# felixyu7/perceiver-io-1

Measured on AMD Instinct MI355X. Metric: samples/sec (whole node) IMDB MLM seq_len=512 at 1/2/4/8 MI355X, higher is better.
Workload: dtype bf16; 1 GPU; mlm256; model=perceiver-io-mlm latents=256x64 layers=3x(1+6) vocab=10003, global_batch=64, seq_len=512, parallelism=dp1, backend=hip, graph=True, allreduce_in_graph=False, bucket_update=False

## Files before the change

perceiver_io_amd/csrc/binding.cpp:

```cpp
#include <torch/extension.h>
#include <ATen/hip/HIPContext.h>
#include <hip/hip_runtime.h>

#include "host_api.h"

#include <tuple>
#include <unordered_map>
#include <vector>

using torch::Tensor;
using OptT = c10::optional<Tensor>;

namespace {
hipStream_t stream() { return at::hip::getCurrentHIPStream(); }

#ifndef PIO_CHECKS
#define PIO_CHECKS 0
#endif
int64_t check_errors(bool reset) {
  return (int64_t)(pio::check_errors_elementwise(reset) | pio::check_errors_optim(reset) |
                   pio::check_errors_mlm_head(reset) | pio::check_errors_mlm_select(reset) |
                   pio::check_errors_ce_head(reset) | pio::check_errors_topk_head(reset) |
                   pio::check_errors_rowgemm(reset) | pio::check_errors_pixel_head(reset) |
                   pio::check_errors_soft_ce_head(reset) | pio::check_errors_augment(reset) |
// ... 1401 lines not shown
  TORCH_CHECK(R > 0 && R < (int64_t(1) << 31), "text_kv_fwd: bad row count");
  TORCH_CHECK(la.size() == 4 && lb.size() == 4, "text_kv_fwd: [lnw, lnb, w, bias] per layer");
  auto opts = E.options();
  Tensor x = torch::empty({B, L, 64}, opts);
  Tensor mean = torch::empty({R}, opts), rstd = torch::empty({R}, opts);
  Tensor kva = torch::empty({R, 128}, opts.dtype(torch::kBFloat16)), kvb = torch::empty({R, 128}, opts.dtype(torch::kBFloat16));
  auto proj = [](std::vector<Tensor>& l, Tensor& kv) {
    TORCH_CHECK(l[0].is_contiguous() && l[0].numel() == 64 && l[1].is_contiguous() && l[1].numel() == 64,
                "text_kv_fwd: LN affine of 64 channels");
    TORCH_CHECK(l[2].dim() == 2 && l[2].is_contiguous() && l[2].size(0) == 128 && l[2].size(1) == 64,
                "text_kv_fwd: w must be (128, 64) contiguous");
    TORCH_CHECK(l[3].is_contiguous() && l[3].numel() == 128, "text_kv_fwd: bias of 128 columns");
    return pio::TextKvProj{f32p(l[0]), f32p(l[1]), bfp(l[2]), f32p(l[3]), bfp_mut(kv)};
  };
  pio::TextKvFwdArgs a{};
  a.ids = ids.data_ptr<int64_t>();
  a.E = f32p(E);
  a.P = f32p(P);
  a.scale = (float)scale;
  a.V = E.size(0);
  a.L = (int)L;
  a.R = (int)R;
  a.eps = (float)eps;
  a.a = proj(la, kva);
  a.b = proj(lb, kvb);
  a.X = x.data_ptr<float>();
  a.mean = mean.data_ptr<float>();
  a.rstd = rstd.data_ptr<float>();
  TORCH_CHECK(pio::text_kv_fwd_launch(a, stream()), "text_kv_fwd: operands must be 16-byte aligned");
  checked_sync("text_kv_fwd");
  return {x, mean, rstd, kva, kvb};
}

Tensor text_kv_bwd(Tensor ga, Tensor gb, Tensor x, Tensor mean, Tensor rstd, std::vector<Tensor> la,
                   std::vector<Tensor> lb, std::vector<Tensor> grads, bool slab, OptT job_slab,
                   std::vector<Tensor> job_dsts, std::vector<int64_t> job_offs) {
  CHECK_CUDA(ga); CHECK_CUDA(x);
  const int64_t R = ga.size(0);
  TORCH_CHECK(ga.dim() == 2 && ga.is_contiguous() && ga.size(1) == 128 && gb.is_contiguous() && gb.dim() == 2 &&
                  gb.size(0) == R && gb.size(1) == 128,
              "text_kv_bwd: dK|dV must be (R, 128) contiguous");
  TORCH_CHECK(x.is_contiguous() && x.numel() == R * 64 && mean.is_contiguous() && mean.numel() == R &&
                  rstd.is_contiguous() && rstd.numel() == R,
              "text_kv_bwd: x (R, 64) and its row statistics");
  TORCH_CHECK(R > 0 && R < kTallRows, "text_kv_bwd: bad row count");
  TORCH_CHECK(!g_det || slab, "deterministic mode: text_kv_bwd parameter gradients need slab mode");
  TORCH_CHECK(la.size() == 3 && lb.size() == 3 && grads.size() == 8, "text_kv_bwd: [lnw, lnb, w] per layer, 8 targets");
  const int64_t sr = slab ? (R + 63) / 64 : 0;
  int vrs = -1;
  auto layer = [&](const Tensor& g, std::vector<Tensor>& l, int t0) {
    TORCH_CHECK(l[0].is_contiguous() && l[0].numel() == 64 && l[1].is_contiguous() && l[1].numel() == 64,
                "text_kv_bwd: LN affine of 64 channels");
    TORCH_CHECK(l[2].dim() == 2 && l[2].is_contiguous() && l[2].size(0) == 128 && l[2].size(1) == 64,
                "text_kv_bwd: w must be (128, 64) contiguous");
    pio::TextKvGrad o{};
    o.G = f32p(g);
    o.lnw = f32p(l[0]);
    o.lnb = f32p(l[1]);
    o.W = bfp(l[2]);
    o.dlnw = vec_target(grads[t0], 64, "dlnw", vrs, sr);
    o.dlnb = vec_target(grads[t0 + 1], 64, "dlnb", vrs, sr);
    o.dW = vec_target(grads[t0 + 2], 128 * 64, "dW", vrs, sr);
    o.db = vec_target(grads[t0 + 3], 128, "db", vrs, sr);
    return o;
  };
  Tensor dx = torch::empty({R, 64}, ga.options());
  pio::TextKvBwdArgs a{};
  a.a = layer(ga, la, 0);
  a.b = layer(gb, lb, 4);
  a.X = f32p(x);
  a.mean = f32p(mean);
  a.rstd = f32p(rstd);
  a.dX = dx.data_ptr<float>();
  a.vrs = vrs < 0 ? 0 : vrs;
  a.slab = slab ? 1 : 0;
  a.R = (int)R;
  a.job = make_job(job_slab, job_dsts, job_offs);
  TORCH_CHECK(pio::text_kv_bwd_launch(a, stream()), "text_kv_bwd: operands must be 16-byte aligned");
  return dx;
}

void embed_bwd(Tensor ids, Tensor g, OptT dE, OptT dP, double scale, OptT job_slab, std::vector<Tensor> job_dsts,
               std::vector<int64_t> job_offs) {
  TORCH_CHECK(g.is_contiguous() && ids.is_contiguous());
  const pio::SlabJob job = make_job(job_slab, job_dsts, job_offs);
  const int B = (int)ids.size(0), L = (int)ids.size(1), C = (int)g.size(2);
  if (dE.has_value()) TORCH_CHECK(dE->is_contiguous() && dE->size(1) == C, "dE must be (V, C) contiguous");
  if (dP.has_value()) TORCH_CHECK(dP->is_contiguous() && dP->size(1) == C && dP->size(0) >= L, "dP must be (>= L, C)");
  if ((!dE.has_value() || dE->size(0) < (1 << 24)) &&
      pio::embed_bwd_local_launch(ids.data_ptr<int64_t>(), f32p(g), dE.has_value() ? dE->data_ptr<float>() : nullptr,
                                  dP.has_value() ? dP->data_ptr<float>() : nullptr, B, L, C, (float)scale, job,
                                  stream()))
    return;
  if (job.slab) pio::slab_reduce_launch(job, stream());
  if (dE.has_value()) {
    TORCH_CHECK(dE->is_contiguous() && dE->size(1) == C, "dE must be (V, C) contiguous");
    const bool small = dE->size(0) <= 32767;
    Tensor keys = small ? ids.reshape({-1}).to(torch::kInt16) : ids.reshape({-1});
    auto sorted = keys.sort();
    Tensor sid = std::get<0>(sorted).to(torch::kInt64).contiguous(), perm = std::get<1>(sorted).contiguous();
    pio::embed_bwd_sorted_launch(sid.data_ptr<int64_t>(), perm.data_ptr<int64_t>(), f32p(g), dE->data_ptr<float>(),
                                 ids.numel(), C, (float)scale, stream());
  }
  if (dP.has_value())
    pio::embed_bwd_launch(ids.data_ptr<int64_t>(), f32p(g), nullptr, dP->data_ptr<float>(), B, L, C, (float)scale,
                          stream());
}

std::vector<Tensor> text_mask(Tensor x, OptT pad, Tensor state, int64_t unk, int64_t mask, double p, int64_t lo,
// ... 802 lines not shown
        py::arg("pre") = std::vector<Tensor>{}, py::arg("post") = std::vector<Tensor>{});
  m.def("sb_bwd", &sb_bwd, py::arg("dz"), py::arg("x0"), py::arg("saved"), py::arg("params"),
        py::arg("scale"), py::arg("eps"), py::arg("pre") = std::vector<Tensor>{},
        py::arg("pre_saved") = std::vector<Tensor>{}, py::arg("zero_out") = py::none(),
        py::arg("post") = std::vector<Tensor>{}, py::arg("post_io") = std::vector<Tensor>{});
  m.def("sb_wgrad", &sb_wgrad, py::arg("jobs"), py::arg("job_slab") = py::none(),
        py::arg("job_dsts") = std::vector<Tensor>(), py::arg("job_offs") = std::vector<int64_t>());
  m.def("post_attn_ln_linear_fwd", &post_attn_ln_linear_fwd, py::arg("o"), py::arg("x"), py::arg("wo"), py::arg("bo"),
        py::arg("g2"), py::arg("be2"), py::arg("eps"), py::arg("w1"), py::arg("b1"), py::arg("w2"), py::arg("b2"),
        py::arg("lnw"), py::arg("lnb"), py::arg("wq"), py::arg("bq"), py::arg("seed") = py::none(),
        py::arg("site") = 0, py::arg("p") = 0.0);
  m.def("ln_linear_post_attn_bwd", &ln_linear_post_attn_bwd, py::arg("g"), py::arg("wq"), py::arg("x"),
        py::arg("mean1"), py::arg("rstd1"), py::arg("lnw"), py::arg("lnb"), py::arg("dres"), py::arg("ll_grads"),
        py::arg("y"), py::arg("m2"), py::arg("r2"), py::arg("u"), py::arg("o"), py::arg("wo"), py::arg("w1"),
        py::arg("w2"), py::arg("g2"), py::arg("be2"), py::arg("H"), py::arg("pa_grads"),
        py::arg("job_slab") = py::none(), py::arg("job_dsts") = std::vector<Tensor>(),
        py::arg("job_offs") = std::vector<int64_t>(), py::arg("seed") = py::none(), py::arg("site") = 0,
        py::arg("p") = 0.0, py::arg("zero_out") = py::none(), py::arg("att_qkv") = py::none(),
        py::arg("att_lse") = py::none(), py::arg("att_out") = py::none(), py::arg("att_scale") = 0.0);
  m.def("post_attn_bwd", &post_attn_bwd, py::arg("dz"), py::arg("y"), py::arg("m2"), py::arg("r2"), py::arg("u"),
        py::arg("o"), py::arg("wo"), py::arg("w1"), py::arg("w2"), py::arg("g2"), py::arg("be2"), py::arg("H"),
        py::arg("grads"), py::arg("slab") = false, py::arg("job_slab") = py::none(),
        py::arg("job_dsts") = std::vector<Tensor>(), py::arg("job_offs") = std::vector<int64_t>(),
        py::arg("seed") = py::none(), py::arg("site") = 0, py::arg("p") = 0.0, py::arg("zero_out") = py::none());
  m.def("ln_linear_bwd", &ln_linear_bwd, py::arg("g"), py::arg("w"), py::arg("x"), py::arg("mean"), py::arg("rstd"),
        py::arg("lnw"), py::arg("lnb"), py::arg("dres"), py::arg("need_dx"), py::arg("dlnw"), py::arg("dlnb"),
        py::arg("dW"), py::arg("db"), py::arg("pe") = py::none(), py::arg("kin") = -1, py::arg("slab") = false,
        py::arg("job_slab") = py::none(), py::arg("job_dsts") = std::vector<Tensor>(),
        py::arg("job_offs") = std::vector<int64_t>(), py::arg("dx_out") = py::none(), py::arg("pe_index") = py::none());
  m.def("text_kv_fwd", &text_kv_fwd, py::arg("ids"), py::arg("E"), py::arg("P"), py::arg("scale"), py::arg("eps"),
        py::arg("la"), py::arg("lb"));
  m.def("text_kv_bwd", &text_kv_bwd, py::arg("ga"), py::arg("gb"), py::arg("x"), py::arg("mean"), py::arg("rstd"),
        py::arg("la"), py::arg("lb"), py::arg("grads"), py::arg("slab") = false, py::arg("job_slab") = py::none(),
        py::arg("job_dsts") = std::vector<Tensor>(), py::arg("job_offs") = std::vector<int64_t>());
  m.def("wgrad", &wgrad, py::arg("g"), py::arg("a"), py::arg("amode"), py::arg("mean"), py::arg("rstd"), py::arg("lnw"),
        py::arg("lnb"), py::arg("rows_per_wg"), py::arg("dW"), py::arg("db"), py::arg("pe") = py::none(),
        py::arg("kin") = -1, py::arg("pe_index") = py::none());
  m.def("mlm_select", &mlm_select, py::arg("labels"), py::arg("cap"), py::arg("gcap"), py::arg("sticky") = py::none(),
        py::arg("queries") = py::none());
  m.def("index_add_rows", &index_add_rows);
  m.def("gather_rows", &gather_rows, py::arg("src"), py::arg("idx"));
  m.def("batch_sum2", &batch_sum2, py::arg("a"), py::arg("b"), py::arg("ob_acc") = py::none());
  m.def("pixel_ce_fwd", &pixel_ce_fwd);
  m.def("pixel_ce_bwd", &pixel_ce_bwd);
  m.def("pixel_predict", &pixel_predict, py::arg("h"), py::arg("w"), py::arg("b"), py::arg("qidx"), py::arg("qvalid"),
        py::arg("Q"), py::arg("npix"), py::arg("labels") = py::none());
  m.def("nonzero_compact", &nonzero_compact, py::arg("img"), py::arg("cap"), py::arg("segs") = 0, py::arg("tile") = 0);
  m.def("event_compact", &event_compact, py::arg("img"), py::arg("lab"), py::arg("words"), py::arg("key_cap"),
        py::arg("query_cap"), py::arg("wmask"), py::arg("ncls"), py::arg("segs") = 0, py::arg("tile") = 0);
  m.def("stage_step", &stage_step, py::arg("dsts"), py::arg("srcs"), py::arg("hyper_dst") = py::none(),
        py::arg("hyper") = std::vector<double>{}, py::arg("seed_dst") = py::none(),
        py::arg("seeds") = std::vector<int64_t>{});
  m.def("ce_fwd", &ce_fwd, py::arg("h"), py::arg("idx"), py::arg("labels"), py::arg("w"), py::arg("bias"),
        py::arg("count"), py::arg("zero_out") = py::none(), py::arg("count_labels") = false);
  m.def("ce_bwd", &ce_bwd, py::arg("h"), py::arg("labels"), py::arg("w"), py::arg("bias"),
        py::arg("lse"), py::arg("gout"), py::arg("count"), py::arg("dH"), py::arg("dW"), py::arg("db"),
        py::arg("accumulate"), py::arg("rowmap") = py::none(), py::arg("slab") = false, py::arg("u") = py::none(),
        py::arg("u_ml") = py::none());
  m.def("vocab_topk", &vocab_topk, py::arg("h"), py::arg("idx"), py::arg("w"), py::arg("bias"), py::arg("k"));
  m.def("soft_ce_fwd", &soft_ce_fwd, py::arg("h"), py::arg("label_a"), py::arg("label_b"), py::arg("lam"), py::arg("w"),
        py::arg("bias"), py::arg("eps"));
  m.def("soft_ce_bwd", &soft_ce_bwd, py::arg("hs"), py::arg("label_a"), py::arg("label_b"), py::arg("lam"), py::arg("w"),
        py::arg("bias"), py::arg("eps"), py::arg("lse"), py::arg("gout"), py::arg("count"), py::arg("dH"), py::arg("dW"),
        py::arg("db"), py::arg("accumulate"));
  m.def("batch_mix", &batch_mix, py::arg("x"), py::arg("y"), py::arg("mix"));
  m.def("batch_augment", &batch_augment, py::arg("src"), py::arg("params"), py::arg("mean"), py::arg("std"),
        py::arg("out_h"), py::arg("out_w"));
// ... 58 lines not shown
```

perceiver_io_amd/csrc/host_api.h:

```cpp
#pragma once
#include <stdint.h>

#include <hip/hip_runtime_api.h>

namespace pio {


struct AttnArgs {
  const uint16_t* q; long long q_bs; int q_rs;
  const uint16_t* k; long long k_bs; int k_rs;
  const uint16_t* v; long long v_bs; int v_rs;
  const uint8_t* kmask;
  int B, H, Nq, Nk;
  float scale_log2;
  float scale;
  uint32_t drop_thresh;
  float drop_scale;
  const int64_t* seedp;
  uint32_t site;
};

struct DropCfg {
  const int64_t* seed;
  uint32_t site;
// ... 104 lines not shown
  float *dlnw, *dlnb, *dW, *db;
  int vrs, wrs, slab;
  int R;
  PeSplit ps;
  SlabJob job;
};
struct TextKvProj {
  const float *lnw, *lnb;
  const uint16_t* W;
  const float* bias;
  uint16_t* KV;
};
struct TextKvFwdArgs {
  const int64_t* ids;
  const float *E, *P;
  float scale;
  long long V;
  int L, R;
  float eps;
  TextKvProj a, b;
  float *X, *mean, *rstd;
};
struct TextKvGrad {
  const float* G;
  const float *lnw, *lnb;
  const uint16_t* W;
  float *dlnw, *dlnb, *dW, *db;
};
struct TextKvBwdArgs {
  TextKvGrad a, b;
  const float *X, *mean, *rstd;
  float* dX;
  int vrs, slab, R;
  SlabJob job;
};
struct WgradArgs {
  RowsIn G; int N;
  RowsIn A; int Kin, amode;
  const float *mean, *rstd, *lnw, *lnb;
  int R;
  int rows_per_wg;
  float *dW, *db;
  int vrs, wrs;
  PeSplit ps;
};
struct PostAttnFwdArgs {
  const uint16_t* O;
  const float* X;
  PostAttnParams p;
  float* Z;
  PostAttnSaved s;
  int R, Rx;
  NextProj next;
  DropCfg dr;
};
struct SaLayerFwdArgs {
  const uint16_t* QKV;
  int N;
  float scale_log2;
  uint16_t* O;
  float* LSE;
  const float* X;
  PostAttnParams p;
  float* Z;
  PostAttnSaved s;
  int R;
// ... 202 lines not shown
                        float eps, uint16_t* y, float* mean, float* rstd, hipStream_t st);
int pe_proj_bwd_blocks(int M);
void pe_proj_bwd_launch(const float* dy, const float* pix, int nc, const float* mean, const float* rstd, int B, int M,
                        int O, float* D, float* part, hipStream_t st);
void persist_set_spin_limit(unsigned n);
unsigned persist_errors(bool reset);
int persist_sync_words(int B);
bool sa_block_fwd_launch(const SABlockFwdArgs& a, hipStream_t st);
int pixel_ce_blocks(long long R);
void pixel_ce_fwd_launch(int C, int K, const float* H, const float* W, const float* bias, const int64_t* labels,
                         const float* wts, long long R, float* part, float* stats, float* loss, hipStream_t st);
void pixel_ce_bwd_launch(int C, int K, const float* H, const float* W, const float* bias, const int64_t* labels,
                         const float* wts, const float* gout, const float* stats, long long R, float* dH, float* part,
                         float* dW, float* db, hipStream_t st);
void pixel_predict_launch(int C, int K, const float* H, const float* W, const float* bias, const int64_t* qidx,
                          const bool* qvalid, const int64_t* labels, long long R, long long Q, long long npix,
                          uint8_t* classes, float* conf, uint8_t* cmap, int* cpart, hipStream_t st);
void nonzero_compact_launch(const float* img, int B, long long npix, long long cap, int S, int V, int* segcount,
                            float* values, int64_t* index, bool* kmask, int* count, hipStream_t st);
unsigned check_errors_pixel_head(bool reset);
void rand_augment_launch(const uint8_t* src, const float* words, uint8_t* out, uint8_t* tmp, int* hist, int B, int H,
                         int W, int C, int N, int fill, hipStream_t st);
unsigned check_errors_randaugment(bool reset);
void ln_linear_fwd_launch(const LnLinearFwdArgs& a, hipStream_t st);
void post_attn_fwd_launch(const PostAttnFwdArgs& a, int C, hipStream_t st);
void post_attn_ln_linear_fwd_launch(const PostAttnFwdArgs& a, int C, hipStream_t st);
bool sa_layer_fwd_launch(const SaLayerFwdArgs& a, hipStream_t st);
void post_attn_bwd_launch(const PostAttnBwdArgs& a, int C, hipStream_t st);
bool ln_linear_post_attn_bwd_launch(const LnLinearPostAttnBwdArgs& a, int C, hipStream_t st);
void ln_linear_bwd_launch(const LnLinearBwdArgs& a, hipStream_t st);
void wgrad_launch(const WgradArgs& a, hipStream_t st);
bool text_kv_fwd_launch(const TextKvFwdArgs& a, hipStream_t st);
bool text_kv_bwd_launch(const TextKvBwdArgs& a, hipStream_t st);
unsigned check_errors_rowgemm(bool reset);
bool sb_fwd_launch(const SBFwdArgs& a, int C, hipStream_t st);
bool sb_bwd_launch(const SBBwdArgs& a, int C, hipStream_t st);
bool sb_wgrad_launch(SBWgradArgs a, int C, const SlabJob& sj, hipStream_t st);
int soft_ce_row_tiles(int M);
void soft_ce_fwd_launch(const SoftCeArgs& a, hipStream_t st);
void soft_ce_bwd_launch(const SoftCeArgs& a, hipStream_t st);
void batch_mix_launch(const float* x, const int64_t* y, const float* mix, float* out, int64_t* yb, float* lam_out, int B,
                      int H, int W, int Ch, hipStream_t st);
unsigned check_errors_soft_ce_head(bool reset);
int vocab_topk_splits(int M, int V);
int vocab_topk_kt(int k);
void vocab_topk_launch(const VocabTopkArgs& a, hipStream_t st);
unsigned check_errors_topk_head(bool reset);

}
```

perceiver_io_amd/csrc/rowgemm.hip:

```cpp
#include "common.h"

namespace pio {

__device__ __forceinline__ float ldf(const float* p) { return *p; }
__device__ __forceinline__ float ldf(const uint16_t* p) { return bf2f(*p); }
__device__ __forceinline__ void stf(float* p, float v) { *p = v; }
__device__ __forceinline__ void stf(uint16_t* p, float v) { *p = f2bf(v); }

template <int MAXT, bool A_KC, bool B_KC>
__device__ __forceinline__ void tile_gemm(const uint16_t* sA, int lda, const uint16_t* sB, int ldb, int BM, int BN,
                                          int K, f32x16 (&acc)[MAXT]) {
  const int w = wave_id();
  const int ntn = BN / 32, nt = (BM / 32) * ntn;
#pragma unroll
  for (int t = 0; t < MAXT; ++t) {
    const int tg = w + 4 * t;
    if (tg < nt) {
      const int m0 = 32 * (tg / ntn), n0 = 32 * (tg % ntn);
      for (int k0 = 0; k0 < K; k0 += 16) {
        const bf16x8 a = A_KC ? frag_kc(sA, lda, m0, k0) : frag_ks(sA, lda, m0, k0);
        const bf16x8 b = B_KC ? frag_kc(sB, ldb, n0, k0) : frag_ks(sB, ldb, n0, k0);
        acc[t] = mfma32(a, b, acc[t]);
      }
    }
// ... 1236 lines not shown
    const float* p = P + (long long)((gr < R ? gr : R - 1) % L) * C + rp_col(j);
    const float4 e0 = *reinterpret_cast<const float4*>(e), e1 = *reinterpret_cast<const float4*>(e + 4);
    const float4 p0 = *reinterpret_cast<const float4*>(p), p1 = *reinterpret_cast<const float4*>(p + 4);
    xv[j][0] = e0.x; xv[j][1] = e0.y; xv[j][2] = e0.z; xv[j][3] = e0.w;
    xv[j][4] = e1.x; xv[j][5] = e1.y; xv[j][6] = e1.z; xv[j][7] = e1.w;
    pv[j][0] = p0.x; pv[j][1] = p0.y; pv[j][2] = p0.z; pv[j][3] = p0.w;
    pv[j][4] = p1.x; pv[j][5] = p1.y; pv[j][6] = p1.z; pv[j][7] = p1.w;
  }
#pragma unroll
  for (int j = 0; j < NCH; ++j)
#pragma unroll
    for (int e = 0; e < 8; ++e) xv[j][e] = __builtin_fmaf(xv[j][e], scale, pv[j][e]);
  row_store<NCH>(xv, X, C, gr, R, C, true);
  float mean, rstd;
  ln_row_stats<NCH>(xv, C, eps, mean, rstd);
  if ((threadIdx.x & 3) == 0 && gr < R) { mean_out[gr] = mean; rstd_out[gr] = rstd; }
  float av[NCH][8];
#pragma unroll
  for (int j = 0; j < NCH; ++j)
#pragma unroll
    for (int e = 0; e < 8; ++e) av[j][e] = ln_affine(xv[j][e], mean, rstd, ga[j][e], ba[j][e]);
  ln_linear_fwd_tile<uint16_t, NCH, true>(av, wa, ga, ba, false, m0, R, C, eps, pa.W, C, pa.bias, N, 0, nullptr, 0, pa.KV,
                                          N, nullptr, nullptr, smem);
#pragma unroll
  for (int j = 0; j < NCH; ++j)
#pragma unroll
    for (int e = 0; e < 8; ++e) av[j][e] = ln_affine(xv[j][e], mean, rstd, gb[j][e], bb[j][e]);
  ln_linear_fwd_tile<uint16_t, NCH, true>(av, wb, gb, bb, false, m0, R, C, eps, pb.W, C, pb.bias, N, 0, nullptr, 0, pb.KV,
                                          N, nullptr, nullptr, smem);
}

constexpr int text_kv_bwd_smem() { return 4 * 64 * 72 * 2 + 16 * 64 * 4 + 4 * 64 * 4; }

__global__ __launch_bounds__(256) void text_kv_bwd_kernel(TextKvGrad la, TextKvGrad lb, const float* __restrict__ X,
                                                          const float* __restrict__ mean,
                                                          const float* __restrict__ rstd, float* __restrict__ dX, int vrs,
                                                          int slab, int R, SlabJob job) {
  constexpr int NCH = 2, C = 64, N = 128, KP = 64, LD = KP + 8, LDG = 64 + 8, LDF = KP + 4;
  extern __shared__ __attribute__((aligned(16))) uint16_t smem[];
  if ((int)blockIdx.x >= (R + 63) / 64) {
    const int jb = (int)blockIdx.x - (R + 63) / 64;
    if (jb < job.nblk) slab_reduce_block(job, jb, reinterpret_cast<float4*>(smem));
    return;
  }
  uint16_t* sG = smem;
  uint16_t* sW = sG + 64 * LDG;
  uint16_t* sXa = sW + 64 * LD;
  uint16_t* sXb = sXa + 64 * LD;
  float* sFa = reinterpret_cast<float*>(sG);
  float* sFb = reinterpret_cast<float*>(sXa);
  float* sPart = reinterpret_cast<float*>(sXb + 64 * LD);
  float* sPb = sPart + 16 * KP;
  const int m0 = blockIdx.x * 64, gr = m0 + rp_row();

  float xv[NCH][8], ga[NCH][8], gb[NCH][8];
  row_load<NCH>(xv, X, C, gr, R, C, true);
  const float mu = *(gr < R ? mean + gr : kZero32B);
  const float rs = *(gr < R ? rstd + gr : kZero32B);
  row_load<NCH>(ga, la.lnw, 0, 0, 1, C, true);
  row_load<NCH>(gb, lb.lnw, 0, 0, 1, C, true);
  float gva[2][8], gvb[2][8];
  bf16x8 wa[NCH], wb[NCH];
  g_fetch<float>(gva, la.G, N, m0, R, 0, N, true);
  tile_fetch<NCH>(wa, la.W, C, 0, N, 64, C, KP, true);
  g_fetch<float>(gvb, lb.G, N, m0, R, 0, N, true);
  tile_fetch<NCH>(wb, lb.W, C, 0, N, 64, C, KP, true);
  {
    float xn[NCH][8];
    row_load<NCH>(xn, la.lnb, 0, 0, 1, C, true);
#pragma unroll
    for (int j = 0; j < NCH; ++j)
#pragma unroll
      for (int e = 0; e < 8; ++e) xn[j][e] += (xv[j][e] - mu) * rs * ga[j][e];
    lds_row_write_bf16<NCH>(sXa, LD, xn);
    row_load<NCH>(xn, lb.lnb, 0, 0, 1, C, true);
#pragma unroll
    for (int j = 0; j < NCH; ++j)
#pragma unroll
      for (int e = 0; e < 8; ++e) xn[j][e] += (xv[j][e] - mu) * rs * gb[j][e];
    lds_row_write_bf16<NCH>(sXb, LD, xn);
  }

  f32x16 acca[1] = {f32x16{}}, accb[1] = {f32x16{}};
  ln_linear_bwd_chunks<float, NCH, 1>(gva, wa, acca, la.G, N, N, la.W, C, C, C, m0, R, true, true, sG, sW, sXa, sPb, la.dW,
                                      la.db, vrs, vrs, slab, 0, 1);
  ln_linear_bwd_chunks<float, NCH, 1>(gvb, wb, accb, lb.G, N, N, lb.W, C, C, C, m0, R, true, true, sG, sW, sXb, sPb, lb.dW,
                                      lb.db, vrs, vrs, slab, 0, 1);
  for_acc<1>(64, KP, [&](int t, int m, int n, int i) {
    sFa[m * LDF + n] = acca[t][i];
    sFb[m * LDF + n] = accb[t][i];
  });
  lds_sync();

  float da[NCH][8], db_[NCH][8];
  lds_row_read<NCH>(da, sFa, LDF);
  lds_row_read<NCH>(db_, sFb, LDF);
  float s1 = 0.f, s2 = 0.f;
#pragma unroll
  for (int j = 0; j < NCH; ++j)
#pragma unroll
    for (int e = 0; e < 8; ++e) {
      xv[j][e] = (xv[j][e] - mu) * rs;
      const float g = da[j][e] * ga[j][e] + db_[j][e] * gb[j][e];
      ga[j][e] = g;
      s1 += g;
      s2 += g * xv[j][e];
    }
  s1 = quad_sum(s1) / C;
  s2 = quad_sum(s2) / C;
#pragma unroll
  for (int j = 0; j < NCH; ++j)
#pragma unroll
    for (int e = 0; e < 8; ++e) ga[j][e] = rs * (ga[j][e] - s1 - xv[j][e] * s2);
  row_store<NCH>(ga, dX, C, gr, R, C, true);
  colsum_partial<NCH>(da, sPart + 4 * KP, KP);
  colsum_partial<NCH>(db_, sPart + 12 * KP, KP);
#pragma unroll
  for (int j = 0; j < NCH; ++j)
#pragma unroll
    for (int e = 0; e < 8; ++e) {
      da[j][e] *= xv[j][e];
      db_[j][e] *= xv[j][e];
    }
  colsum_partial<NCH>(da, sPart, KP);
  colsum_partial<NCH>(db_, sPart + 8 * KP, KP);
  lds_sync();
  colsum_flush(sPart, KP, rep(la.dlnw, vrs, slab), C, slab);
  colsum_flush(sPart + 4 * KP, KP, rep(la.dlnb, vrs, slab), C, slab);
  colsum_flush(sPart + 8 * KP, KP, rep(lb.dlnw, vrs, slab), C, slab);
  colsum_flush(sPart + 12 * KP, KP, rep(lb.dlnb, vrs, slab), C, slab);
}

static void set_smem_once(const void* fn) {
  static const void* done[256] = {nullptr};
  for (auto& d : done) {
    if (d == fn) return;
    if (d == nullptr) {
      (void)hipFuncSetAttribute(fn, hipFuncAttributeMaxDynamicSharedMemorySize, 160 * 1024);
      d = fn;
      return;
    }
  }
}

static bool al16(const void* p) { return (reinterpret_cast<uintptr_t>(p) & 15) == 0; }
static bool av_ok(std::initializer_list<const void*> ptrs, std::initializer_list<long long> widths) {
  for (const void* p : ptrs)
    if (!al16(p)) return false;
  for (long long w : widths)
    if (w & 7) return false;
  return true;
}

static int vec_flags(const void* G, int g_rs, int N, const void* W, int w_rs, int Kin, const float* lnw,
                     const float* lnb) {
  int vf = 0;
  if (G && al16(G) && !(g_rs & 7) && !(N & 7)) vf |= kVecG;
  if (al16(W) && !(w_rs & 7) && w_rs >= Kin) vf |= kVecW;
  if (lnw && al16(lnw) && al16(lnb)) vf |= kVecLn;
  return vf;
}

static int pick_nch(int K) {
// ... 174 lines not shown
static void wgrad_n(int nch, const WgradArgs& a, int rps, hipStream_t st) {
  switch (nch) {
    case 1: wgrad_t<TG, TA, 1>(a, rps, st); break;
    case 2: wgrad_t<TG, TA, 2>(a, rps, st); break;
    case 4: wgrad_t<TG, TA, 4>(a, rps, st); break;
    default: wgrad_t<TG, TA, 5>(a, rps, st); break;
  }
}

void wgrad_launch(const WgradArgs& a, hipStream_t st) {
  const int nblk = (a.N + 63) / 64;
  int rps = a.rows_per_wg;
  if (rps <= 0) {
    const int splits = (512 + nblk - 1) / nblk;
    rps = (a.R + splits - 1) / splits;
  }
  rps = round_up(rps < 64 ? 64 : rps, 64);
  const int nch = pick_nch(a.Kin);
  if (a.G.bf16 && a.A.bf16) wgrad_n<uint16_t, uint16_t>(nch, a, rps, st);
  else if (a.G.bf16) wgrad_n<uint16_t, float>(nch, a, rps, st);
  else if (a.A.bf16) wgrad_n<float, uint16_t>(nch, a, rps, st);
  else wgrad_n<float, float>(nch, a, rps, st);
}

bool text_kv_fwd_launch(const TextKvFwdArgs& a, hipStream_t st) {
  if (a.R <= 0 || a.L <= 0 ||
      !av_ok({a.E, a.P, a.X, a.a.lnw, a.a.lnb, a.a.W, a.a.KV, a.b.lnw, a.b.lnb, a.b.W, a.b.KV}, {}))
    return false;
  hipLaunchKernelGGL(text_kv_fwd_kernel, dim3((a.R + 63) / 64), dim3(256), ln_linear_fwd_smem<2>(), st, a.ids, a.E, a.P,
                     a.scale, a.V, a.L, a.R, a.eps, a.a, a.b, a.X, a.mean, a.rstd);
  return true;
}

bool text_kv_bwd_launch(const TextKvBwdArgs& a, hipStream_t st) {
  if (a.R <= 0 || !av_ok({a.a.G, a.a.lnw, a.a.lnb, a.a.W, a.b.G, a.b.lnw, a.b.lnb, a.b.W, a.X, a.dX}, {})) return false;
  const dim3 grid((a.R + 63) / 64 + (a.job.slab ? a.job.nblk : 0));
  hipLaunchKernelGGL(text_kv_bwd_kernel, grid, dim3(256), text_kv_bwd_smem(), st, a.a, a.b, a.X, a.mean, a.rstd, a.dX,
                     a.vrs, a.slab, a.R, a.job);
  return true;
}

}

namespace pio {
unsigned check_errors_rowgemm(bool reset) { return pio_read_errors(reset); }
}
```

perceiver_io_amd/ops/emulation.py:

```python
from __future__ import annotations

import math
import torch
import torch.nn.functional as F

LOG2E = 1.4426950408889634


def _bf(x):
    return x.to(torch.bfloat16).to(torch.float32)


M32 = 0xFFFFFFFF


def _u32(x):
    return x & M32


def hash3(a, b, c):
    h = _u32(_u32(a * 0x9E3779B1) ^ _u32(b + 0x7F4A7C15))
    h = h ^ _u32(c * 0x85EBCA77)
    h = _u32((h ^ (h >> 15)) * 0x2C1B3C6D)
    h = _u32((h ^ (h >> 12)) * 0x297A2D39)
# ... 721 lines not shown
            step = (n - int(h[nz[-1]])) // 255
            if step == 0:
                continue
            lut = ((step // 2 + (torch.cumsum(h, 0) - h)) // step).clamp(max=255)
            out[..., c] = lut[x[..., c]]
        return out
    return x


def rand_augment(src, words, fill: int = 0):
    B = src.shape[0]
    w = words.detach().to(device=src.device, dtype=torch.float32)
    out = torch.empty_like(src)
    for b in range(B):
        x = src[b].to(torch.int64)
        for l in range(w.shape[1]):
            x = _ra_layer(x, w[b, l], fill)
        out[b] = x.to(torch.uint8)
    return out


def embed_fwd(ids, E, P, scale):
    return E[ids] * scale + P[: ids.shape[1]].unsqueeze(0)


def text_kv_fwd(ids, E, P, scale, eps, la, lb):
    x = embed_fwd(ids, E, P, scale)
    x2 = x.reshape(-1, x.shape[-1])
    kva, mean, rstd = ln_linear_fwd(x2, la[0], la[1], eps, la[2], la[3], 0, None, True, True)
    kvb = ln_linear_fwd(x2, lb[0], lb[1], eps, lb[2], lb[3], 0, None, True, False)[0]
    return [x, mean, rstd, kva, kvb]


def text_kv_bwd(ga, gb, x, mean, rstd, la, lb, grads, slab=False, job_slab=None, job_dsts=(), job_offs=()):
    _run_job(job_slab, job_dsts, job_offs)
    _SLAB[0] = slab
    try:
        xf = x.reshape(-1, x.shape[-1]).float()
        xh = (xf - mean[:, None]) * rstd[:, None]
        g = None
        for G, (lnw, lnb, w), (dlnw, dlnb, dW, db) in ((ga, la, grads[0:4]), (gb, lb, grads[4:8])):
            gf = G.float()
            dxn = _bf(gf) @ _bf(w.float())
            _acc(dW, _bf(gf).t() @ _bf(xh * lnw + lnb))
            _acc(db, gf.sum(0))
            _acc(dlnw, (dxn * xh).sum(0))
            _acc(dlnb, dxn.sum(0))
            g = dxn * lnw if g is None else g + dxn * lnw
        s1 = g.mean(-1, keepdim=True)
        s2 = (g * xh).mean(-1, keepdim=True)
        return rstd[:, None] * (g - s1 - xh * s2)
    finally:
        _SLAB[0] = False


def embed_bwd(ids, g, dE, dP, scale, job_slab=None, job_dsts=(), job_offs=()):
    _run_job(job_slab, job_dsts, job_offs)
    C = g.shape[-1]
    if dE is not None:
        dE.index_add_(0, ids.reshape(-1), g.reshape(-1, C) * scale)
    if dP is not None:
        dP[: ids.shape[1]] += g.sum(0)


def _unit24(h):
    return (h >> 8).to(torch.float32) * (1.0 / 16777216.0)

# ... 520 lines not shown
```

perceiver_io_amd/ops/fused.py:

```python
from __future__ import annotations

import math
import os
from dataclasses import dataclass
from typing import List, Optional

import torch

from . import emulation, ext
from ..parallel.reducer import bucket_ready_point

EPS = 1e-5
WGRAD_SLAB = True
BF16_DQKV = True
ATTN_SLAB = True
CHAIN_ATT = True
TALL_ROWS = 1 << 17


def kernels(t: torch.Tensor):
    return ext.require() if t.is_cuda else emulation


class WeightCache:
# ... 66 lines not shown
                K.slab_reduce(t, ds, os_)

    def run_side():
        with torch.cuda.stream(stream):
            for K, t, ds, os_, _ in side:
                t.record_stream(stream)
                K.slab_reduce(t, ds, os_)

    return run_side


def defer_slab(K, t: torch.Tensor, dsts, offs):
    if not dsts:
        return
    st = torch.cuda.current_stream(t.device) if t.is_cuda else None
    _pending.append((K, t, list(dsts), list(offs), st))
    if not _flush_queued[0]:
        try:
            torch.autograd.Variable._execution_engine.queue_callback(_flush_pending)
            _flush_queued[0] = True
        except RuntimeError:
            _flush_pending()


def _take_job() -> dict:
    if not _pending:
        return {}
    _, t, ds, os_, _ = _pending.pop(0)
    return dict(job_slab=t, job_dsts=ds, job_offs=os_)


class _GradSlab:

    def __init__(self, R: int, sizes, like: torch.Tensor):
        self.offs, P = [], 0
        for n in sizes:
            self.offs.append(P)
            P += (n + 3) // 4 * 4
        self.sizes = list(sizes)
        self.t = torch.empty(((R + 63) // 64, P), dtype=torch.float32, device=like.device)

    def targets(self):
        return [self.t[:, o:o + n] for o, n in zip(self.offs, self.sizes)]

    def defer(self, K, dsts):
        ds, os_ = [], []
        for i, d in enumerate(dsts):
            if d is None:
                continue
            for t, extra in (d if isinstance(d, list) else [(d, 0)]):
                ds.append(t.view(-1))
                os_.append(self.offs[i] + extra)
        defer_slab(K, self.t, ds, os_)


def _grad_of(p: torch.Tensor):
    if not p.requires_grad:
        return None
    if p.grad is None:
        p.grad = torch.zeros_like(p)
    return p.grad


@dataclass(frozen=True)
class LayerSpec:
    cross: bool
    packed: bool
    C: int
    heads: int
    dropout: float


def layer_spec_and_params(layer):
# ... 1045 lines not shown
    return _LayerFn.apply(spec, bw, _seed(p_attn, x_q.device), p_attn, src, x_q, x_kv, kmask, *ps)


def _fusable(layer, x=None) -> bool:
    spec, _ = layer_spec_and_params(layer)
    d = spec.C // spec.heads
    return spec.C in (32, 64, 128) and d in (16, 32, 64, 128)


def can_fuse(layer, x_kv=None) -> bool:
    ch = x_kv.channels if isinstance(x_kv, KVSource) else (x_kv.shape[-1] if x_kv is not None else 0)
    return _fusable(layer) and ch <= 160


def self_attention_layer(layer, x):
    if not _fusable(layer, x):
        return layer.eager_forward(x)
    return _run_layer(layer, x)


def cross_attention_layer(layer, x_q, x_kv, pad_mask=None):
    src = x_kv if isinstance(x_kv, KVSource) else None
    if not can_fuse(layer, x_kv):
        if src is not None:
            x_kv = src.materialize()
        return layer.eager_forward(x_q, x_kv, pad_mask)
    if x_q.dim() == 3 and x_q.shape[0] > 1 and x_q.stride(0) == 0:
        x_q = x_q[:1]
    return _run_layer(layer, x_q, src.x if src is not None else x_kv, pad_mask, src)


TEXT_KV_FUSED = os.environ.get("PERCEIVER_TEXT_KV_FUSED", "1") != "0"
TEXT_KV_C = 64


class _TextEmbedFn(torch.autograd.Function):
    @staticmethod
    def forward(ctx, ids, emb, pos, scale, kvp=None):
        K = kernels(emb)
        ids = ids.contiguous()
        if kvp is not None:
            C = TEXT_KV_C
            la, lb = ([ps[2], ps[3], wkv, ps[5][C:]] for ps, wkv in kvp["layers"])
            out, *kvp["out"] = K.text_kv_fwd(ids, emb, pos[: ids.shape[1]].contiguous(), scale, EPS, la, lb)
        else:
            out = K.embed_fwd(ids, emb, pos[: ids.shape[1]].contiguous(), scale)
        ctx.save_for_backward(ids)
        ctx.scale, ctx.emb, ctx.pos = scale, emb, pos
        return out

    @staticmethod
    def backward(ctx, g):
        (ids,) = ctx.saved_tensors
        K = kernels(g)
        targets = []
        for p, need in ((ctx.emb, ctx.needs_input_grad[1]), (ctx.pos, ctx.needs_input_grad[2])):
            if need and p.grad is None:
                p.grad = torch.zeros_like(p)
            targets.append(p.grad if need else None)
        from . import deterministic

        if deterministic() and g.is_cuda:
            C = g.shape[-1]
            if targets[0] is not None:
                targets[0].index_put_((ids.reshape(-1),), g.reshape(-1, C) * ctx.scale, accumulate=True)
            if targets[1] is not None:
# ... 28 lines not shown
    for cross in (layers[0][0], layers[1][0]):
        if not _fusable(cross):
            return None
        spec, ps = layer_spec_and_params(cross)
        if not (spec.cross and spec.packed and spec.C == C and ps[2].shape[0] == C):
            return None
        out.append((ps, _bf16_weights(spec, ps)[1]))
    return out


def _text_kv_source(ad, ids, layers) -> KVSource:
    kvp = {"layers": layers}
    x = _TextEmbedFn.apply(ids, ad.text_embedding.weight, ad.pos_encoding, float(ad.scale), kvp)
    mean, rstd, kva, kvb = kvp.pop("out")
    src = KVSource(x)
    tk = {"first": id(layers[0][0][0]), "layers": layers}
    for (ps, wkv), kv in zip(layers, (kva, kvb)):
        src.entries[id(ps[0])] = {"kv": kv, "mean": mean, "rstd": rstd, "dkv": None, "factored": False, "wkv": wkv,
                                  "implicit": None, "sb_bwd": False, "tkv": tk, "claim": True}
    tk["ents"] = tuple(src.entries[id(ps[0])] for ps, _ in layers)
    return src


def _text_kv_backward(K, ent, key, x2, mean, rstd, like):
    tk = ent["tkv"]
    if key != tk["first"]:
        return None
    ea, eb = tk["ents"]
    if ea["dkv"] is None or eb["dkv"] is None:
        raise RuntimeError("fused encoder: the text input backward needs the key/value gradients of both layer_1 "
                           "and layer_n")
    C = TEXT_KV_C
    R = x2.shape[0]
    sl = _GradSlab(R, [C, C, 2 * C * C, 2 * C] * 2, like)
    ops, dsts = [], []
    for ps, wkv in tk["layers"]:
        ops.append([ps[2].detach(), ps[3].detach(), wkv])
        flat = [None if _grad_of(p) is None else _grad_of(p).view(-1) for p in (ps[2], ps[3], ps[4], ps[5])]
        dsts += [flat[0], flat[1], None if flat[2] is None else flat[2][C * C:3 * C * C],
                 None if flat[3] is None else flat[3][C:3 * C]]
    dx = K.text_kv_bwd(ea["dkv"].view(R, 2 * C), eb["dkv"].view(R, 2 * C), x2, mean, rstd, ops[0], ops[1],
                       sl.targets(), slab=True, **_take_job())
    sl.defer(K, dsts)
    ea["dkv"] = eb["dkv"] = None
    return dx


def encoder_forward(encoder, x, pad_mask=None):
    from ..models.adapters import ImageInputAdapter, TextInputAdapter

    ad = encoder.input_adapter
    if isinstance(ad, TextInputAdapter):
        kv_layers = _text_kv_layers(encoder, ad, x)
        src = _text_kv_source(ad, x, kv_layers) if kv_layers is not None else KVSource(text_embed(ad, x))
    elif isinstance(ad, ImageInputAdapter) and not x.requires_grad:
        ad.check_shape(x)
        pix = x.reshape(x.shape[0], -1, ad.num_image_channels).float().contiguous()
        src = KVSource(pix, pe=ad.padded_position_encoding(), kin=ad.num_input_channels)
    else:
        src = KVSource(ad(x))
    return _encode(encoder, src, pad_mask)


def encode_inputs(encoder, x_in, pad_mask=None):
    return _encode(encoder, KVSource(x_in.float().contiguous()), pad_mask)


def encode_sparse(encoder, values, index, pad_mask=None):
    ad = encoder.input_adapter
    pix = values.reshape(values.shape[0], values.shape[1], ad.num_image_channels).float().contiguous()
    idx = index if index.dtype == torch.int64 and index.is_contiguous() else index.long().contiguous()
    src = KVSource(pix, pe=ad.padded_position_encoding(), kin=ad.num_input_channels, index=idx)
    return _encode(encoder, src, pad_mask)


# ... 70 lines not shown
```

Measured before the change: 49250 samples/s.

## Let text KV backward workgroups process multiple row tiles with register-held weight grads

Adds an optional multi-tile mode to the fused text key/value backward kernel. In this mode each workgroup loops over several 64-row tiles, keeps its weight, bias and LN-affine gradient partials in registers, and prefetches the next tile while finishing the current one. This shrinks the gradient slab and the later slab reduction. The default tile count resolves to 1, so by default a restructured single-tile kernel runs, and the multi-tile path costs extra registers and less grid parallelism.

```diff
diff --git a/perceiver_io_amd/csrc/binding.cpp b/perceiver_io_amd/csrc/binding.cpp
--- a/perceiver_io_amd/csrc/binding.cpp
+++ b/perceiver_io_amd/csrc/binding.cpp
@@ -1457,9 +1457,13 @@
   return {x, mean, rstd, kva, kvb};
 }
 
+int64_t text_kv_bwd_wgs(int64_t R, int64_t tiles) {
+  TORCH_CHECK(R > 0 && R < kTallRows && tiles >= 0, "text_kv_bwd_wgs: bad row or tile count");
+  return pio::text_kv_bwd_wgs((int)R, (int)tiles);
+}
 Tensor text_kv_bwd(Tensor ga, Tensor gb, Tensor x, Tensor mean, Tensor rstd, std::vector<Tensor> la,
                    std::vector<Tensor> lb, std::vector<Tensor> grads, bool slab, OptT job_slab,
-                   std::vector<Tensor> job_dsts, std::vector<int64_t> job_offs) {
+                   std::vector<Tensor> job_dsts, std::vector<int64_t> job_offs, int64_t tiles) {
   CHECK_CUDA(ga); CHECK_CUDA(x);
   const int64_t R = ga.size(0);
   TORCH_CHECK(ga.dim() == 2 && ga.is_contiguous() && ga.size(1) == 128 && gb.is_contiguous() && gb.dim() == 2 &&
@@ -1471,7 +1475,8 @@
   TORCH_CHECK(R > 0 && R < kTallRows, "text_kv_bwd: bad row count");
   TORCH_CHECK(!g_det || slab, "deterministic mode: text_kv_bwd parameter gradients need slab mode");
   TORCH_CHECK(la.size() == 3 && lb.size() == 3 && grads.size() == 8, "text_kv_bwd: [lnw, lnb, w] per layer, 8 targets");
-  const int64_t sr = slab ? (R + 63) / 64 : 0;
+  TORCH_CHECK(tiles >= 0, "text_kv_bwd: tiles per workgroup must be >= 0");
+  const int64_t sr = slab ? pio::text_kv_bwd_wgs((int)R, (int)tiles) : 0;
   int vrs = -1;
   auto layer = [&](const Tensor& g, std::vector<Tensor>& l, int t0) {
     TORCH_CHECK(l[0].is_contiguous() && l[0].numel() == 64 && l[1].is_contiguous() && l[1].numel() == 64,
@@ -1500,6 +1505,7 @@
   a.vrs = vrs < 0 ? 0 : vrs;
   a.slab = slab ? 1 : 0;
   a.R = (int)R;
+  a.tiles = (int)tiles;
   a.job = make_job(job_slab, job_dsts, job_offs);
   TORCH_CHECK(pio::text_kv_bwd_launch(a, stream()), "text_kv_bwd: operands must be 16-byte aligned");
   return dx;
@@ -2368,7 +2374,9 @@
         py::arg("la"), py::arg("lb"));
   m.def("text_kv_bwd", &text_kv_bwd, py::arg("ga"), py::arg("gb"), py::arg("x"), py::arg("mean"), py::arg("rstd"),
         py::arg("la"), py::arg("lb"), py::arg("grads"), py::arg("slab") = false, py::arg("job_slab") = py::none(),
-        py::arg("job_dsts") = std::vector<Tensor>(), py::arg("job_offs") = std::vector<int64_t>());
+        py::arg("job_dsts") = std::vector<Tensor>(), py::arg("job_offs") = std::vector<int64_t>(),
+        py::arg("tiles") = 1);
+  m.def("text_kv_bwd_wgs", &text_kv_bwd_wgs, py::arg("R"), py::arg("tiles") = 1);
   m.def("wgrad", &wgrad, py::arg("g"), py::arg("a"), py::arg("amode"), py::arg("mean"), py::arg("rstd"), py::arg("lnw"),
         py::arg("lnb"), py::arg("rows_per_wg"), py::arg("dW"), py::arg("db"), py::arg("pe") = py::none(),
         py::arg("kin") = -1, py::arg("pe_index") = py::none());
diff --git a/perceiver_io_amd/csrc/host_api.h b/perceiver_io_amd/csrc/host_api.h
--- a/perceiver_io_amd/csrc/host_api.h
+++ b/perceiver_io_amd/csrc/host_api.h
@@ -160,6 +160,7 @@
   const float *X, *mean, *rstd;
   float* dX;
   int vrs, slab, R;
+  int tiles;
   SlabJob job;
 };
 struct WgradArgs {
@@ -428,6 +429,8 @@
 void wgrad_launch(const WgradArgs& a, hipStream_t st);
 bool text_kv_fwd_launch(const TextKvFwdArgs& a, hipStream_t st);
 bool text_kv_bwd_launch(const TextKvBwdArgs& a, hipStream_t st);
+int text_kv_bwd_tiles(int R);
+int text_kv_bwd_wgs(int R, int tiles);
 unsigned check_errors_rowgemm(bool reset);
 bool sb_fwd_launch(const SBFwdArgs& a, int C, hipStream_t st);
 bool sb_bwd_launch(const SBBwdArgs& a, int C, hipStream_t st);
diff --git a/perceiver_io_amd/csrc/rowgemm.hip b/perceiver_io_amd/csrc/rowgemm.hip
--- a/perceiver_io_amd/csrc/rowgemm.hip
+++ b/perceiver_io_amd/csrc/rowgemm.hip
@@ -1292,14 +1292,53 @@
 
 constexpr int text_kv_bwd_smem() { return 4 * 64 * 72 * 2 + 16 * 64 * 4 + 4 * 64 * 4; }
 
+template <bool MULTI>
+__device__ __forceinline__ void text_kv_bwd_chunks(float (&gv)[2][8], bf16x8 (&wb)[2], f32x16 (&acc)[1],
+                                                   f32x16 (&wacc)[2][1], float (&bacc)[2], const TextKvGrad& g, int m0,
+                                                   int R, uint16_t* sG, uint16_t* sW, const uint16_t* sXn, float* sPb,
+                                                   int vrs, int slab) {
+  constexpr int NCH = 2, C = 64, N = 128, KP = 64, LD = KP + 8, LDG = 64 + 8;
+  const int w = wave_id(), l = lane_id();
+#pragma unroll
+  for (int c = 0; c < 2; ++c) {
+    const int nc = 64 * c;
+    g_store(gv, sG, LDG);
+    tile_store<NCH>(wb, sW, LD, 64, KP);
+    float cs[8];
+#pragma unroll
+    for (int e = 0; e < 8; ++e) cs[e] = gv[0][e] + gv[1][e];
+    lds_sync();
+    if (c == 0) {
+      g_fetch<float>(gv, g.G, N, m0, R, 64, N, true);
+      tile_fetch<NCH>(wb, g.W, C, 64, N, 64, C, KP, true);
+    }
+    tile_gemm<1, true, false>(sG, LDG, sW, LD, 64, KP, 64, acc);
+    if constexpr (MULTI) tile_gemm<1, false, false>(sG, LDG, sXn, LD, 64, KP, 64, wacc[c]);
+    else wgrad_tile<1>(sG, LDG, sXn, LD, 64, KP, N - nc, C, rep(g.dW, vrs, slab) + (long long)nc * C, C, slab);
+#pragma unroll
+    for (int e = 0; e < 8; ++e) {
+      const float s = xor32_sum(xor16_sum(cs[e] + dpp<0x128>(cs[e])));
+      if (l < 8) sPb[w * 64 + 8 * l + e] = s;
+    }
+    lds_sync();
+    if (threadIdx.x < 64) {
+      const int t = threadIdx.x;
+      const float s = sPb[t] + sPb[64 + t] + sPb[128 + t] + sPb[192 + t];
+      if constexpr (MULTI) bacc[c] += s;
+      else gadd(rep(g.db, vrs, slab) + nc + t, s, slab);
+    }
+  }
+}
+
+template <bool MULTI>
 __global__ __launch_bounds__(256) void text_kv_bwd_kernel(TextKvGrad la, TextKvGrad lb, const float* __restrict__ X,
                                                           const float* __restrict__ mean,
                                                           const float* __restrict__ rstd, float* __restrict__ dX, int vrs,
-                                                          int slab, int R, SlabJob job) {
+                                                          int slab, int R, int T, int nwg, SlabJob job) {
   constexpr int NCH = 2, C = 64, N = 128, KP = 64, LD = KP + 8, LDG = 64 + 8, LDF = KP + 4;
   extern __shared__ __attribute__((aligned(16))) uint16_t smem[];
-  if ((int)blockIdx.x >= (R + 63) / 64) {
-    const int jb = (int)blockIdx.x - (R + 63) / 64;
+  if ((int)blockIdx.x >= nwg) {
+    const int jb = (int)blockIdx.x - nwg;
     if (jb < job.nblk) slab_reduce_block(job, jb, reinterpret_cast<float4*>(smem));
     return;
   }
@@ -1311,12 +1350,17 @@
   float* sFb = reinterpret_cast<float*>(sXa);
   float* sPart = reinterpret_cast<float*>(sXb + 64 * LD);
   float* sPb = sPart + 16 * KP;
-  const int m0 = blockIdx.x * 64, gr = m0 + rp_row();
+  const int nt = (R + 63) / 64;
+  int tile = (int)blockIdx.x * T, m0 = tile * 64, gr = m0 + rp_row();
+  f32x16 wacc[2][2][1];
+  float bacc[2][2] = {{0.f, 0.f}, {0.f, 0.f}}, lacc[4] = {0.f, 0.f, 0.f, 0.f};
+#pragma unroll
+  for (int q = 0; q < 4; ++q) wacc[q >> 1][q & 1][0] = f32x16{};
 
   float xv[NCH][8], ga[NCH][8], gb[NCH][8];
   row_load<NCH>(xv, X, C, gr, R, C, true);
-  const float mu = *(gr < R ? mean + gr : kZero32B);
-  const float rs = *(gr < R ? rstd + gr : kZero32B);
+  float mu = *(gr < R ? mean + gr : kZero32B);
+  float rs = *(gr < R ? rstd + gr : kZero32B);
   row_load<NCH>(ga, la.lnw, 0, 0, 1, C, true);
   row_load<NCH>(gb, lb.lnw, 0, 0, 1, C, true);
   float gva[2][8], gvb[2][8];
@@ -1325,70 +1369,126 @@
   tile_fetch<NCH>(wa, la.W, C, 0, N, 64, C, KP, true);
   g_fetch<float>(gvb, lb.G, N, m0, R, 0, N, true);
   tile_fetch<NCH>(wb, lb.W, C, 0, N, 64, C, KP, true);
-  {
-    float xn[NCH][8];
-    row_load<NCH>(xn, la.lnb, 0, 0, 1, C, true);
+  for (int k = 0;; ++k) {
+    {
+      float xn[NCH][8];
+      row_load<NCH>(xn, la.lnb, 0, 0, 1, C, true);
+#pragma unroll
+      for (int j = 0; j < NCH; ++j)
+#pragma unroll
+        for (int e = 0; e < 8; ++e) xn[j][e] += (xv[j][e] - mu) * rs * ga[j][e];
+      lds_row_write_bf16<NCH>(sXa, LD, xn);
+      row_load<NCH>(xn, lb.lnb, 0, 0, 1, C, true);
+#pragma unroll
+      for (int j = 0; j < NCH; ++j)
+#pragma unroll
+        for (int e = 0; e < 8; ++e) xn[j][e] += (xv[j][e] - mu) * rs * gb[j][e];
+      lds_row_write_bf16<NCH>(sXb, LD, xn);
+    }
+    f32x16 acca[1] = {f32x16{}}, accb[1] = {f32x16{}};
+    text_kv_bwd_chunks<MULTI>(gva, wa, acca, wacc[0], bacc[0], la, m0, R, sG, sW, sXa, sPb, vrs, slab);
+    text_kv_bwd_chunks<MULTI>(gvb, wb, accb, wacc[1], bacc[1], lb, m0, R, sG, sW, sXb, sPb, vrs, slab);
+
+    const int tnext = tile + 1;
+    const bool more = MULTI && k + 1 < T && tnext < nt;
+    float xnx[NCH][8], mun = 0.f, rsn = 0.f;
+    if constexpr (MULTI) {
+      const int m1 = more ? tnext * 64 : R, g1 = m1 + rp_row();
+      row_load<NCH>(xnx, X, C, g1, R, C, true);
+      mun = *(g1 < R ? mean + g1 : kZero32B);
+      rsn = *(g1 < R ? rstd + g1 : kZero32B);
+      g_fetch<float>(gva, la.G, N, m1, R, 0, N, true);
+      tile_fetch<NCH>(wa, la.W, C, 0, N, 64, C, KP, true);
+      g_fetch<float>(gvb, lb.G, N, m1, R, 0, N, true);
+      tile_fetch<NCH>(wb, lb.W, C, 0, N, 64, C, KP, true);
+    }
+
+    for_acc<1>(64, KP, [&](int t, int m, int n, int i) {
+      sFa[m * LDF + n] = acca[t][i];
+      sFb[m * LDF + n] = accb[t][i];
+    });
+    lds_sync();
+
+    float da[NCH][8], db_[NCH][8], dx[NCH][8];
+    lds_row_read<NCH>(da, sFa, LDF);
+    lds_row_read<NCH>(db_, sFb, LDF);
+    float s1 = 0.f, s2 = 0.f;
 #pragma unroll
     for (int j = 0; j < NCH; ++j)
 #pragma unroll
-      for (int e = 0; e < 8; ++e) xn[j][e] += (xv[j][e] - mu) * rs * ga[j][e];
-    lds_row_write_bf16<NCH>(sXa, LD, xn);
-    row_load<NCH>(xn, lb.lnb, 0, 0, 1, C, true);
+      for (int e = 0; e < 8; ++e) {
+        xv[j][e] = (xv[j][e] - mu) * rs;
+        const float g = da[j][e] * ga[j][e] + db_[j][e] * gb[j][e];
+        dx[j][e] = g;
+        s1 += g;
+        s2 += g * xv[j][e];
+      }
+    s1 = quad_sum(s1) / C;
+    s2 = quad_sum(s2) / C;
 #pragma unroll
     for (int j = 0; j < NCH; ++j)
 #pragma unroll
-      for (int e = 0; e < 8; ++e) xn[j][e] += (xv[j][e] - mu) * rs * gb[j][e];
-    lds_row_write_bf16<NCH>(sXb, LD, xn);
-  }
-
-  f32x16 acca[1] = {f32x16{}}, accb[1] = {f32x16{}};
-  ln_linear_bwd_chunks<float, NCH, 1>(gva, wa, acca, la.G, N, N, la.W, C, C, C, m0, R, true, true, sG, sW, sXa, sPb, la.dW,
-                                      la.db, vrs, vrs, slab, 0, 1);
-  ln_linear_bwd_chunks<float, NCH, 1>(gvb, wb, accb, lb.G, N, N, lb.W, C, C, C, m0, R, true, true, sG, sW, sXb, sPb, lb.dW,
-                                      lb.db, vrs, vrs, slab, 0, 1);
-  for_acc<1>(64, KP, [&](int t, int m, int n, int i) {
-    sFa[m * LDF + n] = acca[t][i];
-    sFb[m * LDF + n] = accb[t][i];
-  });
-  lds_sync();
-
-  float da[NCH][8], db_[NCH][8];
-  lds_row_read<NCH>(da, sFa, LDF);
-  lds_row_read<NCH>(db_, sFb, LDF);
-  float s1 = 0.f, s2 = 0.f;
-#pragma unroll
-  for (int j = 0; j < NCH; ++j)
-#pragma unroll
-    for (int e = 0; e < 8; ++e) {
-      xv[j][e] = (xv[j][e] - mu) * rs;
-      const float g = da[j][e] * ga[j][e] + db_[j][e] * gb[j][e];
-      ga[j][e] = g;
-      s1 += g;
-      s2 += g * xv[j][e];
-    }
-  s1 = quad_sum(s1) / C;
-  s2 = quad_sum(s2) / C;
-#pragma unroll
-  for (int j = 0; j < NCH; ++j)
-#pragma unroll
-    for (int e = 0; e < 8; ++e) ga[j][e] = rs * (ga[j][e] - s1 - xv[j][e] * s2);
-  row_store<NCH>(ga, dX, C, gr, R, C, true);
-  colsum_partial<NCH>(da, sPart + 4 * KP, KP);
-  colsum_partial<NCH>(db_, sPart + 12 * KP, KP);
-#pragma unroll
-  for (int j = 0; j < NCH; ++j)
-#pragma unroll
-    for (int e = 0; e < 8; ++e) {
-      da[j][e] *= xv[j][e];
-      db_[j][e] *= xv[j][e];
-    }
-  colsum_partial<NCH>(da, sPart, KP);
-  colsum_partial<NCH>(db_, sPart + 8 * KP, KP);
-  lds_sync();
-  colsum_flush(sPart, KP, rep(la.dlnw, vrs, slab), C, slab);
-  colsum_flush(sPart + 4 * KP, KP, rep(la.dlnb, vrs, slab), C, slab);
-  colsum_flush(sPart + 8 * KP, KP, rep(lb.dlnw, vrs, slab), C, slab);
-  colsum_flush(sPart + 12 * KP, KP, rep(lb.dlnb, vrs, slab), C, slab);
+      for (int e = 0; e < 8; ++e) dx[j][e] = rs * (dx[j][e] - s1 - xv[j][e] * s2);
+    row_store<NCH>(dx, dX, C, gr, R, C, true);
+    colsum_partial<NCH>(da, sPart + 4 * KP, KP);
+    colsum_partial<NCH>(db_, sPart + 12 * KP, KP);
+#pragma unroll
+    for (int j = 0; j < NCH; ++j)
+#pragma unroll
+      for (int e = 0; e < 8; ++e) {
+        da[j][e] *= xv[j][e];
+        db_[j][e] *= xv[j][e];
+      }
+    colsum_partial<NCH>(da, sPart, KP);
+    colsum_partial<NCH>(db_, sPart + 8 * KP, KP);
+    lds_sync();
+    if constexpr (MULTI) {
+      if (threadIdx.x < 64) {
+        const int t = threadIdx.x;
+#pragma unroll
+        for (int q = 0; q < 4; ++q) {
+          const float* p = sPart + 4 * q * KP + t;
+          lacc[q] += p[0] + p[KP] + p[2 * KP] + p[3 * KP];
+        }
+      }
+    } else {
+      colsum_flush(sPart, KP, rep(la.dlnw, vrs, slab), C, slab);
+      colsum_flush(sPart + 4 * KP, KP, rep(la.dlnb, vrs, slab), C, slab);
+      colsum_flush(sPart + 8 * KP, KP, rep(lb.dlnw, vrs, slab), C, slab);
+      colsum_flush(sPart + 12 * KP, KP, rep(lb.dlnb, vrs, slab), C, slab);
+    }
+    if (!more) break;
+    if constexpr (MULTI) {
+      lds_sync();
+#pragma unroll
+      for (int j = 0; j < NCH; ++j)
+#pragma unroll
+        for (int e = 0; e < 8; ++e) xv[j][e] = xnx[j][e];
+      mu = mun;
+      rs = rsn;
+      tile = tnext;
+      m0 = tile * 64;
+      gr = m0 + rp_row();
+    }
+  }
+  if constexpr (MULTI) {
+#pragma unroll
+    for (int q = 0; q < 4; ++q) {
+      float* dW = rep(q < 2 ? la.dW : lb.dW, vrs, slab) + (long long)(64 * (q & 1)) * C;
+      for_acc<1>(64, KP, [&](int t, int m, int n, int i) { gadd(dW + m * C + n, wacc[q >> 1][q & 1][t][i], slab); });
+    }
+    if (threadIdx.x < 64) {
+      const int t = threadIdx.x;
+      gadd(rep(la.db, vrs, slab) + t, bacc[0][0], slab);
+      gadd(rep(la.db, vrs, slab) + 64 + t, bacc[0][1], slab);
+      gadd(rep(lb.db, vrs, slab) + t, bacc[1][0], slab);
+      gadd(rep(lb.db, vrs, slab) + 64 + t, bacc[1][1], slab);
+      gadd(rep(la.dlnw, vrs, slab) + t, lacc[0], slab);
+      gadd(rep(la.dlnb, vrs, slab) + t, lacc[1], slab);
+      gadd(rep(lb.dlnw, vrs, slab) + t, lacc[2], slab);
+      gadd(rep(lb.dlnb, vrs, slab) + t, lacc[3], slab);
+    }
+  }
 }
 
 static void set_smem_once(const void* fn) {
@@ -1629,11 +1729,24 @@
   return true;
 }
 
+int text_kv_bwd_tiles(int R) {
+  (void)R;
+  return 1;
+}
+int text_kv_bwd_wgs(int R, int tiles) {
+  const int T = tiles > 0 ? tiles : text_kv_bwd_tiles(R);
+  return ((R + 63) / 64 + T - 1) / T;
+}
+
 bool text_kv_bwd_launch(const TextKvBwdArgs& a, hipStream_t st) {
   if (a.R <= 0 || !av_ok({a.a.G, a.a.lnw, a.a.lnb, a.a.W, a.b.G, a.b.lnw, a.b.lnb, a.b.W, a.X, a.dX}, {})) return false;
-  const dim3 grid((a.R + 63) / 64 + (a.job.slab ? a.job.nblk : 0));
-  hipLaunchKernelGGL(text_kv_bwd_kernel, grid, dim3(256), text_kv_bwd_smem(), st, a.a, a.b, a.X, a.mean, a.rstd, a.dX,
-                     a.vrs, a.slab, a.R, a.job);
+  const int T = a.tiles > 0 ? a.tiles : text_kv_bwd_tiles(a.R), nwg = text_kv_bwd_wgs(a.R, T);
+  const dim3 grid(nwg + (a.job.slab ? a.job.nblk : 0));
+  auto go = [&](auto kernel) {
+    hipLaunchKernelGGL(kernel, grid, dim3(256), text_kv_bwd_smem(), st, a.a, a.b, a.X, a.mean, a.rstd, a.dX, a.vrs,
+                       a.slab, a.R, T, nwg, a.job);
+  };
+  T > 1 ? go(text_kv_bwd_kernel<true>) : go(text_kv_bwd_kernel<false>);
   return true;
 }
 
diff --git a/perceiver_io_amd/ops/emulation.py b/perceiver_io_amd/ops/emulation.py
--- a/perceiver_io_amd/ops/emulation.py
+++ b/perceiver_io_amd/ops/emulation.py
@@ -777,7 +777,12 @@
     return [x, mean, rstd, kva, kvb]
 
 
-def text_kv_bwd(ga, gb, x, mean, rstd, la, lb, grads, slab=False, job_slab=None, job_dsts=(), job_offs=()):
+def text_kv_bwd_wgs(R, tiles=1):
+    T = tiles if tiles > 0 else 1
+    return ((R + 63) // 64 + T - 1) // T
+
+
+def text_kv_bwd(ga, gb, x, mean, rstd, la, lb, grads, slab=False, job_slab=None, job_dsts=(), job_offs=(), tiles=1):
     _run_job(job_slab, job_dsts, job_offs)
     _SLAB[0] = slab
     try:
diff --git a/perceiver_io_amd/ops/fused.py b/perceiver_io_amd/ops/fused.py
--- a/perceiver_io_amd/ops/fused.py
+++ b/perceiver_io_amd/ops/fused.py
@@ -122,13 +122,13 @@
 
 class _GradSlab:
 
-    def __init__(self, R: int, sizes, like: torch.Tensor):
+    def __init__(self, R: int, sizes, like: torch.Tensor, rows: Optional[int] = None):
         self.offs, P = [], 0
         for n in sizes:
             self.offs.append(P)
             P += (n + 3) // 4 * 4
         self.sizes = list(sizes)
-        self.t = torch.empty(((R + 63) // 64, P), dtype=torch.float32, device=like.device)
+        self.t = torch.empty(((R + 63) // 64 if rows is None else rows, P), dtype=torch.float32, device=like.device)
 
     def targets(self):
         return [self.t[:, o:o + n] for o, n in zip(self.offs, self.sizes)]
@@ -1240,6 +1240,7 @@
 
 TEXT_KV_FUSED = os.environ.get("PERCEIVER_TEXT_KV_FUSED", "1") != "0"
 TEXT_KV_C = 64
+TEXT_KV_TILES = int(os.environ.get("PERCEIVER_TEXT_KV_TILES", "0"))
 
 
 class _TextEmbedFn(torch.autograd.Function):
@@ -1334,7 +1335,7 @@
                            "and layer_n")
     C = TEXT_KV_C
     R = x2.shape[0]
-    sl = _GradSlab(R, [C, C, 2 * C * C, 2 * C] * 2, like)
+    sl = _GradSlab(R, [C, C, 2 * C * C, 2 * C] * 2, like, rows=K.text_kv_bwd_wgs(R, TEXT_KV_TILES))
     ops, dsts = [], []
     for ps, wkv in tk["layers"]:
         ops.append([ps[2].detach(), ps[3].detach(), wkv])
@@ -1342,7 +1343,7 @@
         dsts += [flat[0], flat[1], None if flat[2] is None else flat[2][C * C:3 * C * C],
                  None if flat[3] is None else flat[3][C:3 * C]]
     dx = K.text_kv_bwd(ea["dkv"].view(R, 2 * C), eb["dkv"].view(R, 2 * C), x2, mean, rstd, ops[0], ops[1],
-                       sl.targets(), slab=True, **_take_job())
+                       sl.targets(), slab=True, tiles=TEXT_KV_TILES, **_take_job())
     sl.defer(K, dsts)
     ea["dkv"] = eb["dkv"] = None
     return dx
```

Result: no change. 49210 samples/s (-0.1%).
